# christhetree/mod_extraction

Measured on AMD Instinct MI355X. Metric: 44.1 kHz audio-seconds/sec (train step), interwoven ph/fl/ch, higher is better.
Workload: dtype f32

## Files before the change

### mod_extraction_amd/csrc/wgrad_f16.hip

```cpp
#include "conv_common.h"

typedef _Float16 half8 __attribute__((ext_vector_type(8)));
typedef short short4v __attribute__((__vector_size__(4 * sizeof(short))));

__device__ __forceinline__ floatx16 mfma16w(half8 a, half8 b, floatx16 c)
{
    return __builtin_amdgcn_mfma_f32_32x32x16_f16(a, b, c, 0, 0, 0);
}

#define WF_CH 176
#define WF_KS (WF_CH / 16)

struct WgradF16Args {
    const _Float16 *dz_hi, *dz_lo;
    const _Float16 *x_hi, *x_lo;
    float *part;
    int B, H, rows_per_slab, n_slabs;
};

struct TrLane { int off[4]; };
__device__ __forceinline__ TrLane tr_lane_offsets(int tile, int lane)
{
    const int q = (lane & 15) >> 2, p = lane & 3, g1 = (lane >> 4) & 1, h2 = lane >> 5;
    TrLane L;
#pragma unroll
    for (int ph = 0; ph < 4; ++ph) {
        const int swz = ((ph + q) >> 1) & 1;
        L.off[ph] = (8 * h2 + q) * 128 + ((tile ^ swz) * 64) + 32 * g1 + 8 * p;
    }
    return L;
}
__device__ __forceinline__ half8 tr_frag(const unsigned char *img_bytes, int lane_off, int r0)
{
    const unsigned char *ptr = img_bytes + lane_off + r0 * 128;
    const short4v v0 = __builtin_amdgcn_ds_read_tr16_b64_v4i16((short4v __attribute__((address_space(3))) *)ptr);
    const short4v v1 = __builtin_amdgcn_ds_read_tr16_b64_v4i16((short4v __attribute__((address_space(3))) *)(ptr + 512));
    typedef short short8v __attribute__((__vector_size__(8 * sizeof(short))));
    const short8v both = __builtin_shufflevector(v0, v1, 0, 1, 2, 3, 4, 5, 6, 7);
    return __builtin_bit_cast(half8, both);
}

template <int T>
__global__ __launch_bounds__(256, 1) void wgrad_f16x3_kernel(WgradF16Args a)
{
    constexpr int WIN = WF_CH + 12 * T;
    constexpr int QDZ = (WF_CH + 31) / 32, QX = (WIN + 31) / 32;
    constexpr bool PREF = true;
    constexpr int NV = PREF ? 2 * (QDZ + QX) : 1;
    extern __shared__ __attribute__((aligned(16))) unsigned char smem[];
    _Float16 *dzl = reinterpret_cast<_Float16 *>(smem);
    _Float16 *xl = dzl + 2 * WF_CH * 64;

    const int tid = threadIdx.x, lane = tid & 63, wave = __builtin_amdgcn_readfirstlane(tid >> 6);
    const int g = wave & 1, nt = wave >> 1;
    const int id = blockIdx.x;
    const int kh = (id >> 3) % CV_KH;
    const int slab = (id & 7) + 8 * (id / (8 * CV_KH));
    if (slab >= a.n_slabs) return;

    floatx16 acc[CV_KW];
#pragma unroll
    for (int i = 0; i < CV_KW; ++i)
#pragma unroll
        for (int r = 0; r < 16; ++r) acc[i][r] = 0.0f;

    const int row_begin = slab * a.rows_per_slab;
    int row_end = row_begin + a.rows_per_slab;
    if (row_end > a.B * a.H) row_end = a.B * a.H;
    auto row_valid = [&](int rid) {
        const int hx = rid % a.H + kh - 2;
        return hx >= 0 && hx < a.H;
    };
    auto next_iter = [&](int &rid, int &ch) {
        if (++ch < 2) return;
        ch = 0;
        do { ++rid; } while (rid < row_end && !row_valid(rid));
    };

    floatx4 pv[NV];
    const int sv = tid & 7, pos0 = tid >> 3;
    const int g_thr = ((sv >> 1) * CV_PITCH + pos0) * 16 + (sv & 1) * 8;
    const int l_thr = pos0 * 128 + ((sv ^ (((pos0 >> 1) & 1) << 2)) * 16);
    auto load_vec = [&](int k, int rid, int ch) -> floatx4 {
        const int b = rid / a.H, h = rid - b * a.H, w0 = ch * WF_CH;
        floatx4 z = {0.f, 0.f, 0.f, 0.f};
        if (k < 2 * QDZ) {
            const int split = k / QDZ, q = k - split * QDZ;
            if (pos0 + 32 * q < WF_CH) {
                const _Float16 *row = (split ? a.dz_lo : a.dz_hi) + ((size_t)b * a.H + h) * (4 * CV_PITCH * 16) + w0 * 16;
                return *reinterpret_cast<const floatx4 *>(row + g_thr + q * (32 * 16));
            }
        } else {
            const int kk = k - 2 * QDZ, split = kk / QX, q = kk - split * QX;
            const int w = w0 - 6 * T + pos0 + 32 * q;
            if (pos0 + 32 * q < WIN && w >= 0 && w < CV_PITCH) {
                const _Float16 *row = (split ? a.x_lo : a.x_hi) + ((size_t)b * a.H + (h + kh - 2)) * (4 * CV_PITCH * 16) +
                                      (w0 - 6 * T) * 16;
                return *reinterpret_cast<const floatx4 *>(row + g_thr + q * (32 * 16));
            }
        }
        return z;
    };
    auto store_vec = [&](int k, floatx4 val) {
        if (k < 2 * QDZ) {
            const int split = k / QDZ, q = k - split * QDZ;
            if (pos0 + 32 * q < WF_CH)
                *reinterpret_cast<floatx4 *>(reinterpret_cast<unsigned char *>(dzl) + split * (WF_CH * 128) + q * 4096 + l_thr) = val;
        } else {
            const int kk = k - 2 * QDZ, split = kk / QX, q = kk - split * QX;
            if (pos0 + 32 * q < WIN)
                *reinterpret_cast<floatx4 *>(reinterpret_cast<unsigned char *>(xl) + split * (WIN * 128) + q * 4096 + l_thr) = val;
        }
    };

    int rid = row_begin, ch = 0;
    while (rid < row_end && !row_valid(rid)) ++rid;
    if (PREF && rid < row_end) {
#pragma unroll
        for (int q = 0; q < NV; ++q) pv[q] = load_vec(q, rid, ch);
    }
    const unsigned char *dz_h = reinterpret_cast<const unsigned char *>(dzl);
    const unsigned char *dz_l = dz_h + WF_CH * 128;
    const unsigned char *x_h = reinterpret_cast<const unsigned char *>(xl);
    const unsigned char *x_l = x_h + WIN * 128;
    const TrLane la0 = tr_lane_offsets(0, lane), la1 = tr_lane_offsets(1, lane), lb = tr_lane_offsets(nt, lane);
    TrLane lbg;
#pragma unroll
    for (int j = 0; j < 4; ++j) lbg.off[j] = g ? lb.off[(j + 7 * T) & 3] : lb.off[j];
    const int xg_off = g * 7 * T * 128;
    const int lag_off = g ? la1.off[0] : la0.off[0];
    while (rid < row_end) {
        __syncthreads();
        if (PREF) {
#pragma unroll
            for (int q = 0; q < NV; ++q) store_vec(q, pv[q]);
        } else if (!PREF) {
#pragma unroll 4
            for (int k = 0; k < 2 * (QDZ + QX); ++k) store_vec(k, load_vec(k, rid, ch));
        }
        int nrid = rid, nch = ch;
        next_iter(nrid, nch);
        if (PREF && nrid < row_end) {
#pragma unroll
            for (int q = 0; q < NV; ++q) pv[q] = load_vec(q, nrid, nch);
        }
        __syncthreads();
        half8 AL[3], AH[2][3], BH[7], BL[7];
        auto rd_a = [&](const unsigned char *img, int ks, int j) {
            return tr_frag(img + ks * 2048, j == 0 ? la0.off[0] : (j == 1 ? la1.off[0] : lag_off), 0);
        };
        auto rd_b = [&](const unsigned char *img, int ks, int tap) {
            return tap < 6 ? tr_frag(img + ks * 2048 + xg_off, lbg.off[(tap * T) & 3], tap * T)
                           : tr_frag(img + ks * 2048, lb.off[(6 * T) & 3], 6 * T);
        };
#define WF_PIN(N_PAIR, N_MFMA_TAIL, N_DS_TAIL)                                                     \
    _Pragma("unroll") for (int q_ = 0; q_ < (N_PAIR); ++q_) {                                      \
        __builtin_amdgcn_sched_group_barrier(0x008, 1, 0);                                         \
        __builtin_amdgcn_sched_group_barrier(0x100, 1, 0);                                         \
    }                                                                                              \
    if ((N_MFMA_TAIL) > 0) __builtin_amdgcn_sched_group_barrier(0x008, (N_MFMA_TAIL), 0);          \
    if ((N_DS_TAIL) > 0) __builtin_amdgcn_sched_group_barrier(0x100, (N_DS_TAIL), 0);
#pragma unroll
        for (int j = 0; j < 3; ++j) { AL[j] = rd_a(dz_l, 0, j); AH[0][j] = rd_a(dz_h, 0, j); }
#pragma unroll
        for (int t = 0; t < 7; ++t) BH[t] = rd_b(x_h, 0, t);
#pragma unroll
        for (int ks = 0; ks < WF_KS; ++ks) {
            const int p = ks & 1;
            const bool last = ks + 1 == WF_KS;
            __builtin_amdgcn_sched_barrier(0);
            {
#pragma unroll
                for (int u = 0; u < 13; ++u) acc[u] = mfma16w(AL[u < 12 ? (u & 1) : 2], BH[u < 12 ? (u >> 1) : 6], acc[u]);
#pragma unroll
                for (int t = 0; t < 7; ++t) BL[t] = rd_b(x_l, ks, t);
                WF_PIN(13, 0, 1)
            }
            __builtin_amdgcn_sched_barrier(0);
            {
#pragma unroll
                for (int u = 0; u < 13; ++u) acc[u] = mfma16w(AH[p][u < 12 ? (u & 1) : 2], BH[u < 12 ? (u >> 1) : 6], acc[u]);
                if (!last) {
#pragma unroll
                    for (int j = 0; j < 3; ++j) { AL[j] = rd_a(dz_l, ks + 1, j); AH[p ^ 1][j] = rd_a(dz_h, ks + 1, j); }
                    WF_PIN(12, 1, 0)
                }
            }
            __builtin_amdgcn_sched_barrier(0);
            {
#pragma unroll
                for (int u = 0; u < 13; ++u) acc[u] = mfma16w(AH[p][u < 12 ? (u & 1) : 2], BL[u < 12 ? (u >> 1) : 6], acc[u]);
                if (!last) {
#pragma unroll
                    for (int t = 0; t < 7; ++t) BH[t] = rd_b(x_h, ks + 1, t);
                    WF_PIN(13, 0, 1)
                }
            }
            __builtin_amdgcn_sched_barrier(0);
        }
#undef WF_PIN
        rid = nrid;
        ch = nch;
    }
    const int l32 = lane & 31;
#pragma unroll
    for (int i = 0; i < CV_KW; ++i) {
        const int kw = i == 12 ? 6 : 7 * g + (i >> 1), mt = i == 12 ? g : (i & 1);
        float *dst = a.part + ((((size_t)slab * CV_KH + kh) * CV_KW + kw) * 64) * 64;
#pragma unroll
        for (int r = 0; r < 16; ++r) dst[(mt * 32 + mfma_row(r, lane)) * 64 + nt * 32 + l32] = acc[i][r];
    }
}

__global__ __launch_bounds__(256) void wgrad_f16_reduce_kernel(const float *__restrict__ part, int n_slabs,
                                                               const float *__restrict__ scale, float *__restrict__ dW)
{
    __shared__ double sh[4][64][4];
    const int total = CV_TAPS * 64 * 64;
    const int jq = threadIdx.x & 63, kq = threadIdx.x >> 6;
    const int j = (blockIdx.x * 64 + jq) * 4;
    const int k0 = (int)((long long)n_slabs * kq / 4), k1 = (int)((long long)n_slabs * (kq + 1) / 4);
    double s[4] = {0.0, 0.0, 0.0, 0.0};
    const float *src = part + (size_t)k0 * total + j;
    int k = k0;
    for (; k + 4 <= k1; k += 4) {
        floatx4 v[4];
#pragma unroll
        for (int u = 0; u < 4; ++u) v[u] = *reinterpret_cast<const floatx4 *>(src + (size_t)u * total);
#pragma unroll
        for (int u = 0; u < 4; ++u)
#pragma unroll
            for (int e = 0; e < 4; ++e) s[e] += (double)v[u][e];
        src += (size_t)4 * total;
    }
    for (; k < k1; ++k) {
        const floatx4 v = *reinterpret_cast<const floatx4 *>(src);
#pragma unroll
        for (int e = 0; e < 4; ++e) s[e] += (double)v[e];
        src += total;
    }
#pragma unroll
    for (int e = 0; e < 4; ++e) sh[kq][jq][e] = s[e];
    __syncthreads();
    {
        const int e = kq, jj = j + e;
        const double t = ((sh[0][jq][e] + sh[1][jq][e]) + sh[2][jq][e]) + sh[3][jq][e];
        const int ci = jj % 64, co = (jj / 64) % 64, tap = jj / (64 * 64);
        dW[((size_t)co * 64 + ci) * CV_TAPS + tap] = (float)(t * (double)scale[1]);
    }
}

template <int T>
static int launch_wgrad_f16(const WgradF16Args &a, hipStream_t st)
{
    constexpr int WIN = WF_CH + 12 * T;
    const size_t lds = (size_t)(2 * WF_CH * 64 + 2 * WIN * 64) * sizeof(_Float16);
    static MxLdsLatch latch = {};
    if (mx_set_dyn_lds(latch, (const void *)wgrad_f16x3_kernel<T>, lds) != MX_OK) return MX_ERR_LAUNCH;
    const int groups = (a.n_slabs + 7) / 8;
    hipLaunchKernelGGL((wgrad_f16x3_kernel<T>), dim3(groups * 8 * CV_KH), dim3(256), lds, st, a);
    return mx_launch_status();
}

MX_EXPORT int mx_conv_block_wgrad_f16(const void *dz_hi, const void *dz_lo, const void *x_hi, const void *x_lo,
                                      const float *scale, int64_t B, int64_t H, int32_t dilation,
                                      int64_t rows_per_slab, float *part, float *dW, void *stream)
{
    if (!dz_hi || !dz_lo || !x_hi || !x_lo || !scale || !part || !dW || B <= 0 || H <= 0 || rows_per_slab <= 0)
        return MX_ERR_ARG;
    const int64_t n_slabs = (B * H + rows_per_slab - 1) / rows_per_slab;
    if (n_slabs > 1000000) return MX_ERR_UNSUPPORTED;
    WgradF16Args a{(const _Float16 *)dz_hi, (const _Float16 *)dz_lo, (const _Float16 *)x_hi, (const _Float16 *)x_lo, part,
                   (int)B, (int)H, (int)rows_per_slab, (int)n_slabs};
    hipStream_t st = (hipStream_t)stream;
    int rc;
    switch (dilation) {
    case 1: rc = launch_wgrad_f16<1>(a, st); break;
    case 2: rc = launch_wgrad_f16<2>(a, st); break;
    case 4: rc = launch_wgrad_f16<4>(a, st); break;
    case 8: rc = launch_wgrad_f16<8>(a, st); break;
    case 16: rc = launch_wgrad_f16<16>(a, st); break;
    default: return MX_ERR_UNSUPPORTED;
    }
    if (rc != MX_OK) return rc;
    const int total = CV_TAPS * 64 * 64;
    hipLaunchKernelGGL(wgrad_f16_reduce_kernel, dim3((total + 255) / 256), dim3(256), 0, st, part, (int)n_slabs, scale, dW);
    return mx_launch_status();
}
```

Before: 7677.

## Add 16x16x32 MFMA wgrad kernel for large dilations with chunked width

Adds a new weight-gradient kernel, used for dilations of 8 and up, that uses 16x16x32 f16 MFMA fragments instead of 32x32x16. It processes each row in two 192-column chunks, prefetching the next chunk through registers into LDS. Fragment reads are interleaved with the MFMAs under explicit scheduling barriers. The intent is better fragment reuse and less wasted halo compute for large dilations. The cost is a large accumulator footprint (52 floatx4 in AGPRs) with one block per CU, plus extra scheduling complexity.

New measurement: 7676, median of 3. Within noise of the previous version (-0.0%).

```diff
diff --git a/mod_extraction_amd/csrc/wgrad_f16.hip b/mod_extraction_amd/csrc/wgrad_f16.hip
--- a/mod_extraction_amd/csrc/wgrad_f16.hip
+++ b/mod_extraction_amd/csrc/wgrad_f16.hip
@@ -212,6 +212,182 @@
     }
 }
 
+__device__ __forceinline__ int tr_lane_offset16(int c16, int lane)
+{
+    const int q = (lane & 15) >> 2, p = lane & 3, g4 = lane >> 4;
+    return (8 * g4 + q) * 128 + ((c16 ^ ((q >> 1) << 1) ^ (g4 & 1)) * 32) + 8 * p;
+}
+
+template <int N> struct WfChunk { static constexpr int value = N; };
+
+template <int T>
+__global__ __launch_bounds__(256, 1) void wgrad_f16x3_m16_kernel(WgradF16Args a)
+{
+    static_assert(T % 8 == 0, "first rows of the fragments must be multiples of 8");
+    constexpr int CH0 = 192, NKS = CH0 / 32;
+    constexpr int WIN = CH0 + 12 * T;
+    constexpr int QDZ = CH0 / 32, QX = WIN / 32;
+    constexpr int NV = 2 * (QDZ + QX);
+    extern __shared__ __attribute__((aligned(16))) unsigned char smem[];
+    unsigned char *dzl = smem;
+    unsigned char *xl = dzl + 2 * CH0 * 128;
+
+    const int tid = threadIdx.x, lane = tid & 63, wave = __builtin_amdgcn_readfirstlane(tid >> 6);
+    const int g = wave & 1, nt = wave >> 1;
+    const int id = blockIdx.x;
+    const int kh = (id >> 3) % CV_KH;
+    const int slab = (id & 7) + 8 * (id / (8 * CV_KH));
+    if (slab >= a.n_slabs) return;
+
+    floatx4 acc[52];
+#pragma unroll
+    for (int i = 0; i < 52; ++i)
+#pragma unroll
+        for (int r = 0; r < 4; ++r) acc[i][r] = 0.0f;
+
+    const int row_begin = slab * a.rows_per_slab;
+    int row_end = row_begin + a.rows_per_slab;
+    if (row_end > a.B * a.H) row_end = a.B * a.H;
+    auto row_valid = [&](int rid) {
+        const int hx = rid % a.H + kh - 2;
+        return hx >= 0 && hx < a.H;
+    };
+
+    floatx4 pv[NV];
+    const int sv = tid & 7, pos0 = tid >> 3;
+    const int g_thr = ((sv >> 1) * CV_PITCH + pos0) * 16 + (sv & 1) * 8;
+    const int l_thr = pos0 * 128 + ((sv ^ (((pos0 >> 1) & 1) << 2) ^ (((pos0 >> 3) & 1) << 1)) * 16);
+    auto load_vec = [&](int k, int rid, int ch) -> floatx4 {
+        const int b = rid / a.H, h = rid - b * a.H, w0 = ch * CH0;
+        floatx4 z = {0.f, 0.f, 0.f, 0.f};
+        if (k < 2 * QDZ) {
+            const int split = k / QDZ, q = k - split * QDZ;
+            if (q < QDZ - ch) {
+                const _Float16 *row = (split ? a.dz_lo : a.dz_hi) + ((size_t)b * a.H + h) * (4 * CV_PITCH * 16) + w0 * 16;
+                return *reinterpret_cast<const floatx4 *>(row + g_thr + q * (32 * 16));
+            }
+        } else {
+            const int kk = k - 2 * QDZ, split = kk / QX, q = kk - split * QX;
+            const int w = w0 - 6 * T + pos0 + 32 * q;
+            if (q < QX - ch && w >= 0 && w < CV_PITCH) {
+                const _Float16 *row = (split ? a.x_lo : a.x_hi) + ((size_t)b * a.H + (h + kh - 2)) * (4 * CV_PITCH * 16) +
+                                      (w0 - 6 * T) * 16;
+                return *reinterpret_cast<const floatx4 *>(row + g_thr + q * (32 * 16));
+            }
+        }
+        return z;
+    };
+    auto store_vec = [&](int k, floatx4 val, int ch) {
+        if (k < 2 * QDZ) {
+            const int split = k / QDZ, q = k - split * QDZ;
+            if (q < QDZ - ch) *reinterpret_cast<floatx4 *>(dzl + split * (CH0 * 128) + q * 4096 + l_thr) = val;
+        } else {
+            const int kk = k - 2 * QDZ, split = kk / QX, q = kk - split * QX;
+            if (q < QX - ch) *reinterpret_cast<floatx4 *>(xl + split * (WIN * 128) + q * 4096 + l_thr) = val;
+        }
+    };
+
+    int rid = row_begin;
+    while (rid < row_end && !row_valid(rid)) ++rid;
+    if (rid < row_end) {
+#pragma unroll
+        for (int q = 0; q < NV; ++q) pv[q] = load_vec(q, rid, 0);
+    }
+    const unsigned char *dz_h = dzl, *dz_l = dzl + CH0 * 128, *x_h = xl, *x_l = xl + WIN * 128;
+    int la[2][2], lb[2], lbg[2];
+#pragma unroll
+    for (int j = 0; j < 2; ++j)
+#pragma unroll
+        for (int s = 0; s < 2; ++s) la[j][s] = tr_lane_offset16(2 * (j ^ g) + s, lane);
+#pragma unroll
+    for (int s = 0; s < 2; ++s) {
+        lb[s] = tr_lane_offset16(2 * nt + s, lane);
+        lbg[s] = lb[s] ^ ((g * 7 * T) & 8 ? 32 : 0);
+    }
+    const int xg_off = g * 7 * T * 128;
+
+    half8 FA[2][2][2][2];
+    half8 FB[2][2][2];
+    auto rdA = [&](int buf, int ks, int i) {
+        const int sp = i >> 2, j = (i >> 1) & 1, s = i & 1;
+        FA[buf][sp][j][s] = tr_frag((sp ? dz_h : dz_l) + ks * 4096, la[j][s], 0);
+    };
+    auto rdB = [&](int slot, int ks, int t, int i) {
+        const int sp = i >> 1, s = i & 1;
+        const unsigned char *img = (sp ? x_l : x_h) + ks * 4096;
+        FB[slot][sp][s] = t < 6 ? tr_frag(img + xg_off, lbg[s] ^ ((t * T) & 8 ? 32 : 0), t * T)
+                                : tr_frag(img, lb[s] ^ ((6 * T) & 8 ? 32 : 0), 6 * T);
+    };
+    auto mma = [&](int buf, int slot, int t, int m) {
+        const int term = t < 6 ? m >> 3 : m >> 2;
+        const int j = t < 6 ? (m >> 2) & 1 : 0, sa = (m >> 1) & 1, sb = m & 1;
+        const int u = t < 6 ? 8 * t + (m & 7) : 48 + (m & 3);
+        const half8 av = FA[buf][term == 0 ? 0 : 1][j][sa];
+        const half8 bv = FB[slot][term == 2 ? 1 : 0][sb];
+        asm volatile("v_mfma_f32_16x16x32_f16 %0, %1, %2, %0" : "+a"(acc[u]) : "v"(av), "v"(bv));
+    };
+
+    auto kstep = [&](int ks, bool nxt) __attribute__((always_inline)) {
+        const int buf = ks & 1;
+#pragma unroll
+        for (int t = 0; t < 7; ++t) {
+            const int slot = (7 * ks + t) & 1;
+            const int n_mma = t < 6 ? 24 : 12;
+            const int nb = (t < 6 || nxt) ? 4 : 0, na = (nxt && t < 4) ? 2 : 0;
+            const int every = nb + na == 0 ? 99 : n_mma / (nb + na);
+            __builtin_amdgcn_sched_barrier(0);
+#pragma unroll
+            for (int m = 0; m < n_mma; ++m) {
+                mma(buf, slot, t, m);
+                __builtin_amdgcn_sched_barrier(0);
+                if (m % every == 0 && m / every < nb + na) {
+                    const int r = m / every;
+                    if (r < 2) rdB(slot ^ 1, t < 6 ? ks : ks + 1, t < 6 ? t + 1 : 0, r);
+                    else if (r < 2 + na) rdA(buf ^ 1, ks + 1, 2 * t + r - 2);
+                    else rdB(slot ^ 1, t < 6 ? ks : ks + 1, t < 6 ? t + 1 : 0, r - na);
+                    __builtin_amdgcn_sched_barrier(0);
+                }
+            }
+        }
+    };
+    int nrid = rid;
+    auto chunk = [&](auto chunk_no) __attribute__((always_inline)) {
+        constexpr int ch = decltype(chunk_no)::value;
+        __syncthreads();
+#pragma unroll
+        for (int q = 0; q < NV; ++q) store_vec(q, pv[q], ch);
+        if (ch == 0) {
+#pragma unroll
+            for (int q = 0; q < NV; ++q) pv[q] = load_vec(q, rid, 1);
+        } else if (nrid < row_end) {
+#pragma unroll
+            for (int q = 0; q < NV; ++q) pv[q] = load_vec(q, nrid, 0);
+        }
+        __syncthreads();
+#pragma unroll
+        for (int i = 0; i < 8; ++i) rdA(0, 0, i);
+#pragma unroll
+        for (int i = 0; i < 4; ++i) rdB(0, 0, 0, i);
+#pragma unroll
+        for (int ks = 0; ks < NKS - ch; ++ks) kstep(ks, ks + 1 < NKS - ch);
+    };
+    while (rid < row_end) {
+        do { ++nrid; } while (nrid < row_end && !row_valid(nrid));
+        chunk(WfChunk<0>{});
+        chunk(WfChunk<1>{});
+        rid = nrid;
+    }
+    asm volatile("s_nop 7\n\ts_nop 7" ::: "memory");
+    const int l16 = lane & 15, g4 = lane >> 4;
+#pragma unroll
+    for (int i = 0; i < 52; ++i) {
+        const int kw = i < 48 ? 7 * g + (i >> 3) : 6, j = i < 48 ? (i >> 2) & 1 : 0, sa = (i >> 1) & 1, sb = i & 1;
+        float *dst = a.part + ((((size_t)slab * CV_KH + kh) * CV_KW + kw) * 64) * 64;
+#pragma unroll
+        for (int r = 0; r < 4; ++r) dst[(32 * (j ^ g) + 16 * sa + 4 * g4 + r) * 64 + 32 * nt + 16 * sb + l16] = acc[i][r];
+    }
+}
+
 __global__ __launch_bounds__(256) void wgrad_f16_reduce_kernel(const float *__restrict__ part, int n_slabs,
                                                                const float *__restrict__ scale, float *__restrict__ dW)
 {
@@ -253,12 +429,18 @@
 template <int T>
 static int launch_wgrad_f16(const WgradF16Args &a, hipStream_t st)
 {
-    constexpr int WIN = WF_CH + 12 * T;
-    const size_t lds = (size_t)(2 * WF_CH * 64 + 2 * WIN * 64) * sizeof(_Float16);
+    constexpr bool M16 = T >= 8;
+    constexpr int CH = M16 ? 192 : WF_CH, WIN = CH + 12 * T;
+    const size_t lds = (size_t)(2 * CH * 64 + 2 * WIN * 64) * sizeof(_Float16);
     static MxLdsLatch latch = {};
-    if (mx_set_dyn_lds(latch, (const void *)wgrad_f16x3_kernel<T>, lds) != MX_OK) return MX_ERR_LAUNCH;
     const int groups = (a.n_slabs + 7) / 8;
-    hipLaunchKernelGGL((wgrad_f16x3_kernel<T>), dim3(groups * 8 * CV_KH), dim3(256), lds, st, a);
+    if constexpr (M16) {
+        if (mx_set_dyn_lds(latch, (const void *)wgrad_f16x3_m16_kernel<T>, lds) != MX_OK) return MX_ERR_LAUNCH;
+        hipLaunchKernelGGL((wgrad_f16x3_m16_kernel<T>), dim3(groups * 8 * CV_KH), dim3(256), lds, st, a);
+    } else {
+        if (mx_set_dyn_lds(latch, (const void *)wgrad_f16x3_kernel<T>, lds) != MX_OK) return MX_ERR_LAUNCH;
+        hipLaunchKernelGGL((wgrad_f16x3_kernel<T>), dim3(groups * 8 * CV_KH), dim3(256), lds, st, a);
+    }
     return mx_launch_status();
 }
 
```
